# AndrewGYork/rescan_line_sted

Hardware: AMD Instinct MI355X
Metric: simulated frames/s (512x512, 20 RL iters) (higher is better)
Workload: dtype f32; 1 GPU; astronaut 128->512x512 (np.kron x4), point-descan STED PSF 107x107 (2.0x operating point), simulate (H + Philox Poisson) + 20 RL iterations per frame; n_psf=1, rl_iters=20, fft=576x576

## Files before the change

include/rlsted.h:

```cpp
#ifndef RLSTED_H
#define RLSTED_H

#include <stddef.h>
#include <stdint.h>

#ifdef __cplusplus
extern "C" {
#endif

#define RL_OK 0
#define RL_ERR_INVALID -1
#define RL_ERR_HIP -2
#define RL_ERR_UNSUPPORTED -3
#define RL_ERR_STATE -4

#define RL_F32 0
#define RL_F64 1

#define RL_RNG_NONE 0
#define RL_RNG_PHILOX 1

typedef struct rl_ctx rl_ctx;
typedef struct rl_deconv rl_deconv;
typedef struct rl_comm rl_comm;
// ... 46 lines not shown
int rl_deconv_get_noiseless(rl_deconv* h, double* out);
int rl_deconv_get_measurement(rl_deconv* h, double* out);
int rl_deconv_get_estimate(rl_deconv* h, double* out);
int rl_deconv_get_normalization(rl_deconv* h, double* out);

int rl_forward(rl_deconv* h, const double* x, double* out);
int rl_adjoint(rl_deconv* h, const double* y, double* out, int normalize);

int rl_deconv_last_ms(const rl_deconv* h, double* iterate_ms, double* simulate_ms);

int rl_deconv_bench_cycles(rl_deconv* h, int k, int reps, int rng_kind, uint64_t seed, double* total_ms);

int rl_deconv_device_ptr(rl_deconv* h, int which, void** ptr, size_t* n_elements, int* dtype);

int rl_deconv_measurement_written(rl_deconv* h);

int rl_deconv_strategy(const rl_deconv* h, int* separable, int* real_psf_spectrum, int* split_column_pass, int* frame_pairs);

int rl_deconv_object_classes(const rl_deconv* h, int* classes, int* shared_slices, int* slices);

int rl_deconv_simulated_images(const rl_deconv* h, int* images);

int rl_deconv_draws_ahead(const rl_deconv* h, int* slices);

int rl_deconv_unresolved(rl_deconv* h, unsigned long long* count, int reset);

int rl_deconv_dims(const rl_deconv* h, int* batch, int* n_psf, int* ny, int* nx);

typedef struct rl_task {
    const double* object;
    double total_brightness;
    uint64_t seed;
    uint32_t image_id;
} rl_task;
int rl_batch_run(rl_deconv* h, const rl_task* tasks, int n_tasks, int k_iters, int rng_kind, double* estimates_out);

int rl_batch_submit(rl_deconv* h, const rl_task* tasks, int n_tasks, int k_iters, int rng_kind, void* dev_out, int out_dtype);

#define RL_TRACE_FIELDS 6
int rl_batch_submit_checkpoints(rl_deconv* h, const rl_task* tasks, int n_tasks, const int* k_list, int n_k, int rng_kind,
                                void* const* dev_out, int out_dtype, double* const* trace_dev);

int rl_device_alloc(rl_ctx* ctx, size_t bytes, void** dev_out);
int rl_device_free(rl_ctx* ctx, void* dev);
int rl_device_download(rl_ctx* ctx, const void* dev, int dtype, size_t n_elements, double* host_out);
int rl_device_upload(rl_ctx* ctx, void* dev, int dtype, size_t n_elements, const double* host);
// ... 132 lines not shown
```

rescan_line_sted_amd/_lib.py:

```python
import ctypes
import os

import numpy as np

_HERE = os.path.dirname(os.path.abspath(__file__))
LIB_PATH = os.environ.get('RLSTED_LIB') or os.path.join(_HERE, '_lib', 'librlsted.so')
DEFAULT_DEVICE = int(os.environ.get('RLSTED_DEVICE', '0'))

RL_F32, RL_F64 = 0, 1
RNG_NONE, RNG_PHILOX = 0, 1
DTYPES = {'f32': RL_F32, 'float32': RL_F32, 'f64': RL_F64, 'float64': RL_F64}
RL_ACCEL_NONE, RL_ACCEL_BIGGS_ANDREWS = 0, 1
ACCELERATIONS = {None: RL_ACCEL_NONE, 'none': RL_ACCEL_NONE, 'biggs-andrews': RL_ACCEL_BIGGS_ANDREWS}
RL_STOP_DISCREPANCY, RL_STOP_RELATIVE = 1, 2
STOP_RULES = {'discrepancy': RL_STOP_DISCREPANCY, 'relative': RL_STOP_RELATIVE}


def accel_mode(acceleration):
    try:
        return ACCELERATIONS[acceleration]
    except (KeyError, TypeError):
        raise ValueError("acceleration must be None or 'biggs-andrews'; got %r" % (acceleration,)) from None


# ... 33 lines not shown
    'rl_deconv_get_alpha': (_i, [_vp, _dp]),
    'rl_deconv_set_tv': (_i, [_vp, _c.c_double, _c.c_double]),
    'rl_deconv_get_tv': (_i, [_vp, _dp, _dp]),
    'rl_deconv_divergence': (_i, [_vp, _dp]),
    'rl_deconv_iterate_until': (_i, [_vp, _i, _i, _i, _c.c_double, _c.POINTER(_i), _dp, _c.POINTER(_i)]),
    'rl_deconv_get_object': (_i, [_vp, _dp]),
    'rl_deconv_get_noiseless': (_i, [_vp, _dp]),
    'rl_deconv_get_measurement': (_i, [_vp, _dp]),
    'rl_deconv_get_estimate': (_i, [_vp, _dp]),
    'rl_deconv_get_normalization': (_i, [_vp, _dp]),
    'rl_forward': (_i, [_vp, _dp, _dp]),
    'rl_adjoint': (_i, [_vp, _dp, _dp, _i]),
    'rl_deconv_last_ms': (_i, [_vp, _dp, _dp]),
    'rl_deconv_bench_cycles': (_i, [_vp, _i, _i, _i, _c.c_uint64, _dp]),
    'rl_deconv_time_kernels': (_i, [_vp, _i, _dp]),
    'rl_deconv_time_cycle': (_i, [_vp, _i, _i, _c.c_uint64, _dp, _dp, _dp]),
    'rl_deconv_device_ptr': (_i, [_vp, _i, _c.POINTER(_vp), _c.POINTER(_c.c_size_t), _c.POINTER(_i)]),
    'rl_host_alloc': (_i, [_c.c_size_t, _c.POINTER(_vp)]),
    'rl_host_free': (_i, [_vp]),
    'rl_deconv_strategy': (_i, [_vp, _c.POINTER(_i), _c.POINTER(_i), _c.POINTER(_i), _c.POINTER(_i)]),
    'rl_deconv_object_classes': (_i, [_vp, _c.POINTER(_i), _c.POINTER(_i), _c.POINTER(_i)]),
    'rl_deconv_simulated_images': (_i, [_vp, _c.POINTER(_i)]),
    'rl_deconv_draws_ahead': (_i, [_vp, _c.POINTER(_i)]),
    'rl_deconv_unresolved': (_i, [_vp, _c.POINTER(_c.c_uint64), _i]),
    'rl_deconv_dims': (_i, [_vp, _c.POINTER(_i), _c.POINTER(_i), _c.POINTER(_i), _c.POINTER(_i)]),
    'rl_batch_run': (_i, [_vp, _vp, _i, _i, _i, _dp]),
    'rl_batch_submit': (_i, [_vp, _vp, _i, _i, _i, _vp, _i]),
    'rl_batch_submit_checkpoints': (_i, [_vp, _vp, _i, _c.POINTER(_i), _i, _i, _c.POINTER(_vp), _i, _c.POINTER(_vp)]),
    'rl_device_alloc': (_i, [_vp, _c.c_size_t, _c.POINTER(_vp)]),
    'rl_device_free': (_i, [_vp, _vp]),
    'rl_device_download': (_i, [_vp, _vp, _i, _c.c_size_t, _dp]),
    'rl_device_upload': (_i, [_vp, _vp, _i, _c.c_size_t, _dp]),
    'rl_comm_gather_device': (_i, [_vp, _vp, _c.POINTER(_c.c_size_t), _i, _i, _vp]),
    'rl_comm_bcast_host': (_i, [_vp, _dp, _c.c_size_t, _i]),
    'rl_comm_unique_id': (_i, [_vp]),
    'rl_comm_create': (_i, [_vp, _i, _i, _vp, _c.POINTER(_vp)]),
    'rl_comm_destroy': (_i, [_vp]),
    'rl_comm_info': (_i, [_vp, _c.POINTER(_i), _c.POINTER(_i)]),
    'rl_comm_barrier': (_i, [_vp]),
    'rl_comm_allreduce_max': (_i, [_vp, _dp]),
    'rl_gather': (_i, [_vp, _vp, _i, _i, _c.POINTER(_i), _dp]),
    'rl_gather_device': (_i, [_vp, _vp, _i, _i, _c.POINTER(_i), _c.POINTER(_vp), _c.POINTER(_c.c_size_t), _c.POINTER(_i)]),
    'rl_comm_gather_host': (_i, [_vp, _dp, _c.POINTER(_c.c_size_t), _i, _dp]),
    'rl_rotate_image': (_i, [_vp, _dp, _dp, _i, _i, _c.c_double, _i]),
    'rl_fig3_scan': (_i, [_vp, _vp, _dp, _dp, _c.POINTER(_i), _i, _c.POINTER(_i), _i, _dp, _dp, _dp, _dp]),
    'rl_gauss_fit': (_i, [_dp, _i, _dp, _c.POINTER(_i)]),
# ... 162 lines not shown
        return {'ly': ly.value, 'lx': lx.value, 'pitch': pitch.value, 'device_bytes': nbytes.value}

    def strategy(self):
        a, b, c, d = _i(), _i(), _i(), _i()
        check(lib.rl_deconv_strategy(self.handle, ctypes.byref(a), ctypes.byref(b), ctypes.byref(c), ctypes.byref(d)))
        return {'separable': a.value == 1, 'direct_stencil': a.value == 2, 'real_psf_spectrum': bool(b.value),
                'split_column_pass': bool(c.value), 'frame_pairs': bool(d.value)}

    def object_classes(self):
        a, b, c = _i(), _i(), _i()
        check(lib.rl_deconv_object_classes(self.handle, ctypes.byref(a), ctypes.byref(b), ctypes.byref(c)))
        return {'classes': a.value, 'shared_slices': b.value, 'slices': c.value}

    def simulated_images(self):
        a = _i()
        check(lib.rl_deconv_simulated_images(self.handle, ctypes.byref(a)))
        return a.value

    def draws_ahead(self):
        a = _i()
        check(lib.rl_deconv_draws_ahead(self.handle, ctypes.byref(a)))
        return a.value

    def set_object(self, obj, total_brightness=None):
        obj = as_f64(obj).reshape(self.B, self.ny, self.nx)
        tb = None
        if total_brightness is not None:
            tb = as_f64(np.broadcast_to(np.asarray(total_brightness, dtype=np.float64), (self.B,)))
        check(lib.rl_deconv_set_object(self.handle, ptr(obj), ptr(tb) if tb is not None else None))

    def simulate(self, seed=0, rng=RNG_PHILOX):
        check(lib.rl_deconv_simulate(self.handle, rng, _c.c_uint64(seed)))

    def unresolved(self, reset=False):
        n = _c.c_uint64(0)
        check(lib.rl_deconv_unresolved(self.handle, _c.byref(n), 1 if reset else 0))
        return int(n.value)

    def set_measurement(self, noisy):
        noisy = as_f64(noisy).reshape(self.B, self.V, self.ny, self.nx)
        check(lib.rl_deconv_set_measurement(self.handle, ptr(noisy)))

    def measurement_written(self):
        check(lib.rl_deconv_measurement_written(self.handle))

    def iterate(self, k=1):
# ... 175 lines not shown
```

rescan_line_sted_amd/csrc/aux_kernels.hip:

```cpp
#include <hip/hip_runtime.h>
#include <type_traits>
#include "aux_kernels.hpp"
#include "philox_poisson.hpp"

namespace rl {

template <typename T>
__global__ void k_fill(T* p, size_t n, T value) {
    for (size_t i = (size_t)blockIdx.x * blockDim.x + threadIdx.x; i < n; i += (size_t)gridDim.x * blockDim.x) p[i] = value;
}

__global__ void k_psf_dft_rows(const double* __restrict__ psf, const double2* __restrict__ wx, double2* __restrict__ s1,
                               int py, int px, int lx, int kx) {
    const int k = blockIdx.x * blockDim.x + threadIdx.x;
    const int a = blockIdx.y, v = blockIdx.z;
    if (k >= kx) return;
    const int cx = (px - 1) / 2;
    const double* row = psf + ((size_t)v * py + a) * px;
    double re = 0.0, im = 0.0;
    for (int b = 0; b < px; ++b) {
        const int off = ((b - cx) % lx + lx) % lx;
        const double2 w = wx[(int)(((long long)k * off) % lx)];
        re += row[b] * w.x;
        im += row[b] * w.y;
    }
    s1[((size_t)v * py + a) * kx + k] = make_double2(re, im);
// ... 2 lines not shown
template <typename T>
__global__ void k_psf_dft_cols(const double2* __restrict__ s1, const double2* __restrict__ wy, cx<T>* __restrict__ out,
                               int py, int ly, int kx, int pitch, double scale, int transposed) {
    const int k = blockIdx.x * blockDim.x + threadIdx.x;
    const int ky = blockIdx.y, v = blockIdx.z;
    if (k >= pitch) return;
    const int cy = (py - 1) / 2;
    double re = 0.0, im = 0.0;
    if (k < kx) {
        for (int a = 0; a < py; ++a) {
            const int off = ((a - cy) % ly + ly) % ly;
            const double2 w = wy[(int)(((long long)ky * off) % ly)];
            const double2 s = s1[((size_t)v * py + a) * kx + k];
            re += s.x * w.x - s.y * w.y;
            im += s.x * w.y + s.y * w.x;
        }
    }
    if (transposed) {
        if (k < kx) out[((size_t)v * kx + k) * ly + ky] = mk<T>((T)(re * scale), (T)(im * scale));
    } else {
        out[((size_t)v * ly + ky) * pitch + k] = mk<T>((T)(re * scale), (T)(im * scale));
    }
}

struct PoissonKeys {
    unsigned long long seed0;
    unsigned image0, V;
    const unsigned long long* frame_seeds;
    const unsigned* frame_ids;
    const unsigned* rate_frame;
    __device__ __forceinline__ unsigned long long seed(unsigned img) const { return frame_seeds ? frame_seeds[img / V] : seed0; }
    __device__ __forceinline__ unsigned image(unsigned img) const {
        return frame_seeds ? frame_ids[img / V] * V + img % V : image0 + img;
    }
    template <typename T>
    __device__ __forceinline__ T rate(const T* __restrict__ noiseless, unsigned i, unsigned n_pix) const {
        if (!rate_frame) return noiseless[i];
        const unsigned img = i / n_pix, pix = i - img * n_pix;
        return noiseless[((size_t)rate_frame[img / V] * V + img % V) * n_pix + pix];
    }
    template <typename T>
    __device__ __forceinline__ const T* image_rates(const T* __restrict__ noiseless, unsigned img, unsigned n_pix) const {
        return noiseless + (rate_frame ? (size_t)rate_frame[img / V] * V + img % V : (size_t)img) * n_pix;
    }
};

constexpr int kPoissonE = 8, kPoissonTile = 256 * kPoissonE;
template <typename T, bool TILE_IMG>
__global__ void __launch_bounds__(256) k_poisson(const T* __restrict__ noiseless, T* __restrict__ noisy, unsigned n_pix, unsigned total,
                                                 PoissonKeys keys, int rng_kind) {
    __shared__ unsigned lst_idx[2][kPoissonTile];
    __shared__ T lst_lam[2][kPoissonTile];
    __shared__ unsigned cnt[2], cnt_small;
    const unsigned tid = threadIdx.x;
    const unsigned n_tiles = (total + (unsigned)kPoissonTile - 1u) / (unsigned)kPoissonTile;
    const unsigned turn = (unsigned)((float)gridDim.x * 0.6180339887f) | 1u;
    for (unsigned first = 0, round = 0; first < n_tiles; first += gridDim.x, ++round) {
        const unsigned tile = first + (blockIdx.x + round * turn) % gridDim.x;
        if (tile >= n_tiles) continue;
        const unsigned tile0 = tile * (unsigned)kPoissonTile;
        if (tid == 0) cnt[0] = cnt_small = 0;
        __syncthreads();
        const unsigned img_t = TILE_IMG ? tile0 / n_pix : 0u;
        const T* __restrict__ rates_t = TILE_IMG ? keys.image_rates(noiseless, img_t, n_pix) : nullptr;
#pragma unroll
        for (int e = 0; e < kPoissonE; ++e) {
            const unsigned i = tile0 + tid + 256u * (unsigned)e;
            if (i < total) {
// ... 35 lines not shown
                double k;
                const bool done = philox_ptrs_attempt((double)lam_t, (unsigned)seed, (unsigned)(seed >> 32), keys.image(img), pix, blk, &k);
                if (done || last) {
                    noisy[i] = (T)((done || k >= 0.0 ? k : 0.0) + 1e-9);
                } else {
                    const unsigned q2 = atomicAdd(&cnt[cur ^ 1], 1u);
                    lst_idx[cur ^ 1][q2] = i;
                    lst_lam[cur ^ 1][q2] = lam_t;
                }
            }
            __syncthreads();
            n = cnt[cur ^ 1];
            cur ^= 1;
        }
        for (unsigned q = tid; q < n_small; q += 256u) {
            const unsigned at = kPoissonTile - 1u - q, i = lst_idx[0][at];
            const unsigned img = TILE_IMG ? img_t : i / n_pix;
            noisy[i] = (T)(philox_poisson((double)lst_lam[0][at], keys.seed(img), keys.image(img), i - img * n_pix) + 1e-9);
        }
        __syncthreads();
    }
}

template <typename T>
__global__ void __launch_bounds__(1024) k_frame_sums(const T* __restrict__ x, size_t n, double* __restrict__ out) {
    __shared__ double part[16];
    const size_t chunks = gridDim.y, len = (n + chunks - 1) / chunks, i0 = blockIdx.y * len, i1 = i0 + len < n ? i0 + len : n;
    const T* f = x + (size_t)blockIdx.x * n;
    double v = 0.0;
    for (size_t i = i0 + threadIdx.x; i < i1; i += blockDim.x) v += (double)f[i];
    for (int off = 32; off > 0; off >>= 1) v += __shfl_down(v, off, 64);
    if ((threadIdx.x & 63) == 0) part[threadIdx.x >> 6] = v;
    __syncthreads();
    if (threadIdx.x < 64) {
        v = threadIdx.x < (blockDim.x >> 6) ? part[threadIdx.x] : 0.0;
        for (int off = 8; off > 0; off >>= 1) v += __shfl_down(v, off, 64);
        if (threadIdx.x == 0) out[(size_t)blockIdx.x * chunks + blockIdx.y] = v;
    }
}
template <typename T>
static void frame_sums(const T* x, size_t n, size_t frames, double* sums, hipStream_t s) {
    if (n >= ((size_t)1 << 20) && frames * kSumChunks <= 8192) {
        double* part = sums + frames;
        k_frame_sums<T><<<dim3((unsigned)frames, kSumChunks), 1024, 0, s>>>(x, n, part);
        k_frame_sums<double><<<dim3((unsigned)frames, 1), 64, 0, s>>>(part, (size_t)kSumChunks, sums);
    } else {
// ... 66 lines not shown
    const unsigned g = blocks_for(n, 256);
    if (dtype == DT_F32) k_split_real<float><<<g, 256, 0, s>>>((const cx<float>*)z, n, (float*)re, stats);
    else k_split_real<double><<<g, 256, 0, s>>>((const cx<double>*)z, n, (double*)re, stats);
    return hipGetLastError();
}

template <typename T>
__global__ void k_box_norm(const double* __restrict__ integ, T* __restrict__ out, int V, int py, int px, int ny, int nx) {
    const int j = blockIdx.x * blockDim.x + threadIdx.x, i = blockIdx.y;
    if (j >= nx) return;
    out[(size_t)i * nx + j] = box_norm_pixel<T>(integ, V, py, px, ny, nx, i, j);
}

hipError_t aux_box_norm(int dtype, const double* integral_dev, void* out, int V, int py, int px, int ny, int nx, hipStream_t s) {
    const dim3 grid((unsigned)((nx + 255) / 256), (unsigned)ny);
    if (dtype == DT_F32) k_box_norm<float><<<grid, 256, 0, s>>>(integral_dev, (float*)out, V, py, px, ny, nx);
    else k_box_norm<double><<<grid, 256, 0, s>>>(integral_dev, (double*)out, V, py, px, ny, nx);
    return hipGetLastError();
}

hipError_t aux_poisson(int dtype, const void* noiseless, void* noisy, unsigned n_pix, unsigned n_img, unsigned image0,
                       unsigned long long seed, int rng_kind, void* list_ws, hipStream_t s,
                       const unsigned long long* frame_seeds, const unsigned* frame_ids, unsigned V, const unsigned* rate_frame,
                       unsigned grid_cap) {
    (void)list_ws;
    const PoissonKeys keys{seed, image0, V ? V : 1u, frame_seeds, frame_ids, rate_frame};
    const size_t total = (size_t)n_pix * n_img;
    if (total >= 0xffffffffull - (size_t)kPoissonTile * kPoissonGrid) return hipErrorInvalidValue;
    if (total == 0) return hipSuccess;
    const size_t tiles = (total + kPoissonTile - 1) / kPoissonTile;
    const size_t cap = grid_cap < 1 ? 1 : grid_cap > kPoissonGrid ? kPoissonGrid : grid_cap;
    const unsigned g = (unsigned)(tiles > cap ? cap : tiles);
    const bool tile_img = n_pix % (unsigned)kPoissonTile == 0;
    auto launch = [&](auto zero, auto in_image) {
        using T = decltype(zero);
        k_poisson<T, decltype(in_image)::value><<<g, 256, 0, s>>>((const T*)noiseless, (T*)noisy, n_pix, (unsigned)total, keys, rng_kind);
    };
    if (dtype == DT_F32) tile_img ? launch(0.0f, std::true_type{}) : launch(0.0f, std::false_type{});
    else tile_img ? launch(0.0, std::true_type{}) : launch(0.0, std::false_type{});
    return hipGetLastError();
}

hipError_t aux_scale_convert(int dtype, const double* src, void* dst, size_t n, size_t frames, const double* target,
                             double* sums, hipStream_t s, bool want_sums) {
    if (target || want_sums) frame_sums<double>(src, n, frames, sums, s);
    const unsigned g = blocks_for(n * frames, 256);
    if (dtype == DT_F32) k_scale_convert<float><<<g, 256, 0, s>>>(src, (float*)dst, n, frames, target, sums);
    else k_scale_convert<double><<<g, 256, 0, s>>>(src, (double*)dst, n, frames, target, sums);
    return hipGetLastError();
}

template <typename T>
__global__ void k_any_negative(const T* __restrict__ x, size_t n, int* __restrict__ flag) {
    bool neg = false;
    for (size_t i = (size_t)blockIdx.x * blockDim.x + threadIdx.x; i < n; i += (size_t)gridDim.x * blockDim.x) neg = neg || x[i] < (T)0;
// ... 81 lines not shown
```

rescan_line_sted_amd/csrc/aux_kernels.hpp:

```cpp
#pragma once
#include "fft_core.hpp"

#include <cstddef>

#if defined(__HIPCC__) || defined(__HIP_PLATFORM_AMD__)
#include <hip/hip_runtime.h>
#include "kernel_table.hpp"
#endif

namespace rl {

template <typename T>
RL_HD T box_norm_pixel(const double* __restrict__ integ, int V, int py, int px, int ny, int nx, int i, int j) {
    const int cy = (py - 1) / 2, cx = (px - 1) / 2;
    const int a0 = i + cy - ny + 1 > 0 ? i + cy - ny + 1 : 0, a1 = (i + cy < py - 1 ? i + cy : py - 1) + 1;
    const int b0 = j + cx - nx + 1 > 0 ? j + cx - nx + 1 : 0, b1 = (j + cx < px - 1 ? j + cx : px - 1) + 1;
    double acc = 0.0;
    if (a1 > a0 && b1 > b0) {
        for (int v = 0; v < V; ++v) {
            const double* I = integ + (size_t)v * (py + 1) * (px + 1);
            const double s = (I[(size_t)a1 * (px + 1) + b1] - I[(size_t)a0 * (px + 1) + b1]) - (I[(size_t)a1 * (px + 1) + b0] - I[(size_t)a0 * (px + 1) + b0]);
            acc += s > 0.0 ? s : 0.0;
        }
    }
    return (T)acc;
}

#if defined(__HIPCC__) || defined(__HIP_PLATFORM_AMD__)
hipError_t aux_fill(int dtype, void* p, size_t n, double value, hipStream_t s);
hipError_t aux_psf_spectrum(int dtype, const double* psf_dev, const void* wx_dev, const void* wy_dev, void* s1_dev,
                            void* out, int n_psf, int py, int px, int ly, int lx, int kx, int pitch, int transposed,
                            hipStream_t s);
size_t aux_poisson_workspace_bytes(size_t total_pixels);
constexpr unsigned kPoissonGrid = 4096;
hipError_t aux_poisson(int dtype, const void* noiseless, void* noisy, unsigned n_pix, unsigned n_img, unsigned image0,
                       unsigned long long seed, int rng_kind, void* list_ws, hipStream_t s,
                       const unsigned long long* frame_seeds = nullptr, const unsigned* frame_ids = nullptr, unsigned V = 1,
                       const unsigned* rate_frame = nullptr, unsigned grid_cap = kPoissonGrid);
constexpr size_t kSumChunks = 64;
inline size_t aux_sums_elems(size_t frames) { return frames * (1 + kSumChunks); }
hipError_t aux_scale_convert(int dtype, const double* src, void* dst, size_t n, size_t frames, const double* target,
                             double* sums, hipStream_t s, bool want_sums = false);
hipError_t aux_any_negative(int dtype, const void* src, size_t n, int* flag, hipStream_t s);
hipError_t aux_image_sums(int dtype, const void* src, size_t n, size_t frames, double* sums, hipStream_t s);
hipError_t aux_scale_convert_indexed(int dtype, const double* src, const unsigned* idx, size_t n_unique, void* dst, size_t n, size_t frames,
                                     const double* target, double* sums, hipStream_t s);
hipError_t aux_to_f64(int dtype, const void* src, double* dst, size_t total, hipStream_t s);
hipError_t aux_cast(int dtype_src, const void* src, int dtype_dst, void* dst, size_t total, hipStream_t s);
hipError_t aux_gather_images(int dtype, const void* src, void* dst, const unsigned* list, size_t n, size_t images, unsigned V, hipStream_t s);
hipError_t aux_split_real(int dtype, const void* z, size_t n, void* re, double* stats, hipStream_t s);
hipError_t aux_box_norm(int dtype, const double* integral_dev, void* out, int V, int py, int px, int ny, int nx, hipStream_t s);
#endif
}
```

rescan_line_sted_amd/csrc/philox_poisson.hpp:

```cpp
#pragma once
#include <stdint.h>
#include "fft_core.hpp"

#if defined(__clang__)
#define RL_FP_STRICT _Pragma("clang fp contract(off)")
#else
#define RL_FP_STRICT
#endif

namespace rl {

struct Philox4 {
    uint32_t x[4];
};

RL_HD Philox4 philox4x32_10(uint32_t c0, uint32_t c1, uint32_t c2, uint32_t c3, uint32_t k0, uint32_t k1) {
    const uint32_t M0 = 0xD2511F53u, M1 = 0xCD9E8D57u, W0 = 0x9E3779B9u, W1 = 0xBB67AE85u;
#pragma unroll
    for (int r = 0; r < 10; ++r) {
        const uint64_t p0 = (uint64_t)M0 * c0, p1 = (uint64_t)M1 * c2;
        const uint32_t hi0 = (uint32_t)(p0 >> 32), lo0 = (uint32_t)p0;
        const uint32_t hi1 = (uint32_t)(p1 >> 32), lo1 = (uint32_t)p1;
        c0 = hi1 ^ c1 ^ k0;
        c1 = lo1;
// ... 65 lines not shown
    p = p * r + 1.0;
    p = p * r + 1.0;
    DblBits b;
    b.u = (uint64_t)(1023 + (int)n) << 52;
    return p * b.d;
}

RL_HD double det_logfact(double k) {
    RL_FP_STRICT
    if (k < 20.5) {
        double f = 1.0;
        for (int i = 2; i <= (int)k; ++i) f = f * (double)i;
        return det_log(f);
    }
    const double x = k + 1.0;
    const double xi = 1.0 / x, x2 = xi * xi;
    double c = -1.0 / 1680.0;
    c = c * x2 + 1.0 / 1260.0;
    c = c * x2 - 1.0 / 360.0;
    c = c * x2 + 1.0 / 12.0;
    return ((x - 0.5) * det_log(x) - x) + 0.9189385332046727 + c * xi;
}

RL_HD bool philox_poisson_fast(double lam, uint64_t seed, uint32_t image, uint32_t pixel, double* out) {
    RL_FP_STRICT
    if (!(lam > 0.0)) {
        *out = 0.0;
        return true;
    }
    if (lam < 10.0) return false;
    const uint32_t k0 = (uint32_t)seed, k1 = (uint32_t)(seed >> 32);
    const double slam = __builtin_sqrt(lam);
    const double b = 0.931 + 2.53 * slam;
    const double a = -0.059 + 0.02483 * b;
    const double vr = 0.9277 - 3.6224 / (b - 2.0);
    const Philox4 o = philox4x32_10(pixel, image, 0u, 0x504F4953u, k0, k1);
    const double U = u53(o.x[0], o.x[1]) - 0.5;
    const double V = u53(o.x[2], o.x[3]);
    const double us = 0.5 - (U < 0.0 ? -U : U);
    const double k = __builtin_floor((2.0 * a / us + b) * U + lam + 0.43);
    *out = k;
    return us >= 0.07 && V <= vr;
}

RL_HD bool philox_ptrs_attempt(double lam, uint32_t k0, uint32_t k1, uint32_t image, uint32_t pixel, uint32_t blk, double* kout) {
    RL_FP_STRICT
    const double slam = __builtin_sqrt(lam);
    const double b = 0.931 + 2.53 * slam;
    const double a = -0.059 + 0.02483 * b;
    const double vr = 0.9277 - 3.6224 / (b - 2.0);
    const Philox4 o = philox4x32_10(pixel, image, blk, 0x504F4953u, k0, k1);
    const double U = u53(o.x[0], o.x[1]) - 0.5;
    const double V = u53(o.x[2], o.x[3]);
    const double us = 0.5 - (U < 0.0 ? -U : U);
    const double k = __builtin_floor((2.0 * a / us + b) * U + lam + 0.43);
    *kout = k;
    if (us >= 0.07 && V <= vr) return true;
    if (k < 0.0 || (us < 0.013 && V > us)) return false;
    if (!(V > 0.0)) return true;
    const double invalpha = 1.1239 + 1.1328 / (b - 3.4);
    const double loglam = det_log(lam);
    const double lhs = (det_log(V) + det_log(invalpha)) - det_log(a / (us * us) + b);
    const double rhs = (k * loglam - lam) - det_logfact(k);
    return lhs <= rhs;
}

constexpr uint32_t kPoissonMaxBlocks = 64;

RL_HD double philox_poisson(double lam, uint64_t seed, uint32_t image, uint32_t pixel) {
    RL_FP_STRICT
    const uint32_t k0 = (uint32_t)seed, k1 = (uint32_t)(seed >> 32);
    if (!(lam > 0.0)) return 0.0;
    if (lam < 10.0) {
        const double enlam = det_exp(-lam);
        double X = 0.0, prod = 1.0;
        for (uint32_t blk = 0; blk < kPoissonMaxBlocks; ++blk) {
            const Philox4 o = philox4x32_10(pixel, image, blk, 0x504F4953u, k0, k1);
            prod = prod * u53(o.x[0], o.x[1]);
            if (!(prod > enlam)) return X;
            X = X + 1.0;
            prod = prod * u53(o.x[2], o.x[3]);
            if (!(prod > enlam)) return X;
            X = X + 1.0;
        }
        return X;
    }
    double k = 0.0;
// ... 7 lines not shown
```

rescan_line_sted_amd/csrc/rlsted.cpp:

```cpp
#include "../../include/rlsted.h"

#include <hip/hip_runtime.h>

#include <cmath>
#include <cstdio>
#include <cstdlib>
#include <algorithm>
#include <cstring>
#include <map>
#include <string>
#include <vector>

#include "accel_kernels.hpp"
#include "aux_kernels.hpp"
#include "checkpoint_kernels.hpp"
#include "conv_kernels.hpp"
#include "cycle_schedule.hpp"
#include "kernel_table.hpp"
#include "object_classes.hpp"
#include "ctx.hpp"
#include "sep_kernels.hpp"
#include "sep_taps.hpp"
#include "stop_kernels.hpp"
#include "tv_kernels.hpp"
// ... 23 lines not shown

const KernelTable* table_for(int L) {
    switch (L) {
        case 64: return table_64();
        case 192: return table_192();
        case 256: return table_256();
        case 576: return table_576();
        case 1152: return table_1152();
        case 2304: return table_2304();
        case 4608: return table_4608();
    }
    return nullptr;
}
const int kLengths[] = {64, 192, 256, 576, 1152, 2304, 4608};

size_t esize(int dtype) { return dtype == RL_F32 ? 4 : 8; }

struct PlanOptions {
    bool chunk_mb_set = false;
    double chunk_mb = 0;
    int lanes = 2;
    bool draw_ahead = false;
    int draw_grid = 128;
    bool inplace = true;
    int col_order = 4;
    bool pair = false;
    double pair_max_ratio = 4.0;
    bool sub_one = false;
    int fuse_views = -1;
    bool col_split = true;
    bool real_psf = true;
    bool ones_shortcut = true;
    bool share_objects = true;
    int sep = 1;
    int sep_one = 1;
    int direct = 1;
    bool q_exp_est_set = false, q_exp_ratio_set = false;
    int q_exp_est = 14, q_exp_ratio = 14;
};

PlanOptions plan_options(int dtype, int n_psf) {
    PlanOptions o;
    auto flag = [](const char* name, bool unset) {
        const char* s = getenv(name);
        return s ? atoi(s) != 0 : unset;
    };
    auto number = [](const char* name, int unset, bool* set = nullptr) {
        const char* s = getenv(name);
        if (set) *set = s != nullptr;
        return s ? atoi(s) : unset;
    };
    if (const char* s = getenv("RLSTED_CHUNK_MB")) {
        o.chunk_mb_set = true;
        o.chunk_mb = atof(s);
    }
    o.lanes = std::min(std::max(number("RLSTED_LANES", o.lanes), 1), kMaxLanes);
    o.draw_ahead = flag("RLSTED_DRAW_AHEAD", o.draw_ahead);
    o.draw_grid = std::min(std::max(number("RLSTED_DRAW_GRID", o.draw_grid), 1), (int)kPoissonGrid);
    o.inplace = flag("RLSTED_INPLACE", o.inplace);
    o.col_order = std::max(number("RLSTED_COL_ORDER", o.col_order), 1);
    o.pair = flag("RLSTED_PAIR", dtype == RL_F32 && n_psf == 1);
    if (const char* s = getenv("RLSTED_PAIR_MAX_RATIO")) o.pair_max_ratio = atof(s);
    o.sub_one = flag("RLSTED_SUB_ONE", dtype == RL_F32 && RL_SPEC_QUANT == 0);
    if (const char* s = getenv("RLSTED_FUSE_VIEWS")) o.fuse_views = atoi(s) != 0 ? 1 : 0;
    o.col_split = flag("RLSTED_COL_SPLIT", o.col_split);
    o.real_psf = flag("RLSTED_REAL_PSF", o.real_psf);
    o.ones_shortcut = flag("RLSTED_ONES_SHORTCUT", o.ones_shortcut);
    o.share_objects = flag("RLSTED_SHARE_OBJECTS", o.share_objects);
    o.sep = number("RLSTED_SEP", o.sep);
    o.sep_one = number("RLSTED_SEP_ONE", o.sep_one);
    o.direct = number("RLSTED_DIRECT", o.direct);
    o.q_exp_est = number("RLSTED_Q_EXP_EST", o.q_exp_est, &o.q_exp_est_set);
    o.q_exp_ratio = number("RLSTED_Q_EXP_RATIO", o.q_exp_ratio, &o.q_exp_ratio_set);
    return o;
}

struct TempBuffers {
    std::vector<void*> bufs;
    int get(void** p, size_t bytes) {
        HIP_TRY(hipMalloc(p, bytes));
        bufs.push_back(*p);
// ... 665 lines not shown
    }
    int forward_slice(int f0, int nf) { return forward_frames(f0, nf, off(obj, (size_t)f0 * n_img()), off(noiseless, (size_t)f0 * V * n_img())); }
    int forward_frames(int f0, int nf, const void* x, void* out) {
        if (sep) return sep_forward(x, out, off(sep_tmp(), (size_t)f0 * V * n_img()), nf);
        void* sb = off(spec_b, (size_t)f0 * V * n_spec() * 2);
        void* sa = !pair ? off(spec_a, (size_t)f0 * n_spec() * 2) : sb;
        return forward_pass(x, out, nf, sa, sb, col_split() ? parked(f0) : nullptr);
    }
    std::vector<int> obj_class;
    int n_classes = 0;
    std::vector<SliceShare> share_slices;
    int share_cf = 0;
    std::vector<uint32_t> share_reps, share_rate;
    struct ShareLists { const unsigned *rep_frames, *rate_of; };
    ShareLists share_lists{nullptr, nullptr};
    unsigned* share_dev = nullptr;
    void *obj_c = nullptr, *noiseless_c = nullptr;
    void *cls_spec_a = nullptr, *cls_spec_b = nullptr, *cls_spec_x = nullptr;
    size_t share_cap = 0;
    int share_classes = 0;
    int last_sim_images = 0;
    bool noiseless_sparse = false;
    int last_shared_slices = 0, last_slices = 0;
    int last_draws_ahead = 0;
    bool share_possible() const { return opt.share_objects && !sep && (int)obj_class.size() == B && n_classes < B; }
    size_t layout_share(int cf) {
        share_cf = 0;
        noiseless_sparse = false;
        share_classes = 0;
        share_layout(obj_class, cf, share_slices, share_reps, share_rate);
        return (size_t)class_layout(obj_class, cf, share_slices, share_reps, share_rate);
    }
    int build_share(int cf, const ShareLists* staged) { return place_share(cf, layout_share(cf), staged); }
    int place_share(int cf, size_t total, const ShareLists* staged) {
        if (total > share_cap) {
            HIP_TRY(hipDeviceSynchronize());
            share_cap = 0;
            RL_TRY(release(&obj_c));
            RL_TRY(release(&noiseless_c));
            RL_TRY(release(&cls_spec_a));
            RL_TRY(release(&cls_spec_b));
            RL_TRY(release(&cls_spec_x));
            const size_t cap = (total + 7) / 8 * 8, sp = n_spec() * 2 * esize(dtype);
            RL_TRY(alloc(&obj_c, cap * n_img() * esize(dtype), SLACK));
            RL_TRY(alloc(&noiseless_c, cap * V * n_img() * esize(dtype), SLACK));
            if (!pair_layout) RL_TRY(alloc(&cls_spec_a, cap * sp, SLACK));
// ... 76 lines not shown
        return RL_OK;
    }
    struct Run { int k; bool restart; const Draw* draw; const Checkpoints* cp; int cf; };
    hipStream_t stream_of(int s) const { return s == kCtxStream ? ctx->stream : lane[s].stream; }
    hipEvent_t event_of(const StreamOp& op) const {
        const Lane& l = lane[op.lane];
        switch (op.event) {
            case EventKind::FORK: return fork;
            case EventKind::RATES_READY: return rates_ready;
            case EventKind::DONE: return l.done;
            case EventKind::DRAWN: return l.drawn;
            case EventKind::BEGUN: return l.begun;
            case EventKind::DRAWN_AHEAD: return l.drawn_ahead;
            case EventKind::NONE: break;
        }
        return nullptr;
    }
    int draw_slice(const Draw& d, int sl, int f0, int nf, bool shared, bool ahead) {
        void* ws = ahead ? nullptr : (char*)slice_ws + (size_t)sl * slice_ws_stride;
        TimedScope t(this, TK_POISSON, false);
        const hipError_t e = aux_poisson(dtype, shared ? noiseless_c : off(noiseless, (size_t)f0 * V * n_img()), off(meas, (size_t)f0 * V * n_img()),
                                         (unsigned)n_img(), (unsigned)(nf * V), (unsigned)(f0 * V), d.seed, d.rng_kind, ws, cur(),
                                         d.key_seeds ? d.key_seeds + f0 : nullptr, d.key_ids ? d.key_ids + f0 : nullptr, (unsigned)V,
                                         shared ? share_lists.rate_of + f0 : nullptr, ahead ? (unsigned)opt.draw_grid : (unsigned)kPoissonGrid);
        return e == hipSuccess ? RL_OK : fail(RL_ERR_HIP, std::string("Poisson kernels: ") + hipGetErrorString(e));
    }
    int loop_slice(const Run& r, int f0, int nf) {
        const int k = r.k;
        const bool restart = r.restart;
        const bool shortcut = restart && opt.ones_shortcut && spec_ones && k > 0 && !sep;
        const bool ones_first = shortcut && !accel && !tv_on();
        if (restart && !ones_first) RL_TRY(start_estimate_chunk(f0, nf, !shortcut));
        const bool drop = pair && k >= 4;
        int cp_next = 0;
        for (int i = 0; i < k; ++i) {
            if (accel) RL_TRY(accel_step(f0, nf, acc_steps + i, shortcut && i == 0, restart && i == 0));
            else if (tv_on()) RL_TRY(tv_iterate({f0, nf, shortcut && i == 0, restart && i == 0,  pair}, i > 0 || tv_sum_valid, true));
            else RL_TRY(iterate_chunk({f0, nf, shortcut && i == 0, restart && i == 0, drop && i == k - 1, ones_first && i == 0}));
            if (r.cp && cp_next < r.cp->n_k && r.cp->k_list[cp_next] == i + 1) RL_TRY(take_checkpoint(*r.cp, cp_next++, f0, nf));
        }
        return RL_OK;
    }
    int enqueue(const StreamOp& op, const Run& r) {
        const int f0 = op.slice * r.cf, nf = f0 + r.cf <= B ? r.cf : B - f0;
        active = stream_of(op.stream);
        switch (op.op) {
            case OpKind::WAIT: HIP_TRY(hipStreamWaitEvent(active, event_of(op), 0)); return RL_OK;
// ... 21 lines not shown
        in.share_classes = share_classes;
        in.share_slices = share_slices.data();
        in.draw_ahead = opt.draw_ahead;
        in.cycle_follows = cycle_follows;
        in.before = cycle_state;
        cycle_schedule(in, schedule);
        if (schedule.forks) RL_TRY(ensure_lanes());
        if (draw) {
            const size_t stride = (aux_poisson_workspace_bytes((size_t)cf * V * n_img()) + 255) / 256 * 256;
            if (slice_ws_bytes < stride * schedule.slices) {
                HIP_TRY(hipDeviceSynchronize());
                slice_ws_bytes = 0;
                RL_TRY(release(&slice_ws));
                RL_TRY(alloc(&slice_ws, stride * schedule.slices));
                slice_ws_bytes = stride * schedule.slices;
            }
            slice_ws_stride = stride;
        }
        struct ActiveGuard {
            hipStream_t& a;
            ~ActiveGuard() { a = nullptr; }
        } active_guard{active};
        const Run run{k, restart, draw, cp, cf};
        int rc = RL_OK;
        for (const StreamOp& op : schedule.ops) {
            if (rc != RL_OK && !op.join) continue;
            const int r = enqueue(op, run);
            if (rc == RL_OK) rc = r;
        }
        active = nullptr;
        if (rc != RL_OK) {
            const std::string keep = rl::last_error();
            if (!schedule.joins) (void)join_lanes();
            cycle_state = CycleState{};
            rl::last_error() = keep;
            return rc;
        }
        cycle_state = schedule.after;
        if (draw) {
            last_draws_ahead = schedule.draws_ahead;
            noiseless_sparse = schedule.shared_slices > 0;
            last_shared_slices = schedule.shared_slices;
            last_slices = schedule.slices;
            last_sim_images = schedule.sim_images;
        }
        if (restart) {
            est_ready = true;
            spec_valid = true;
            iterations = 0;
        }
        if (pair && k >= 4) spec_valid = false;
        if (accel) {
            spec_valid = false;
            acc_steps += k;
        }
        if (tv_on()) spec_valid = false;
        if (k > 0 || restart) tv_sum_valid = tv_on() && !accel && k > 0;
        iterations += k;
        return RL_OK;
    }
};

namespace rl {
// ... 602 lines not shown
}


int rl_deconv_strategy(const rl_deconv* h, int* separable, int* real_psf_spectrum, int* split_column_pass, int* frame_pairs) {
    if (!h) return fail(RL_ERR_INVALID, "handle is NULL");
    if (frame_pairs) *frame_pairs = h->pair ? 1 : 0;
    if (separable) *separable = h->sep ? (h->sep_direct ? 2 : 1) : 0;
    if (real_psf_spectrum) *real_psf_spectrum = h->psf_hat_re ? 1 : 0;
    if (split_column_pass) *split_column_pass = !h->sep && !h->pair && h->col_split() ? 1 : 0;
    return RL_OK;
}

int rl_deconv_object_classes(const rl_deconv* h, int* classes, int* shared_slices, int* slices) {
    if (!h) return fail(RL_ERR_INVALID, "handle is NULL");
    if (classes) *classes = (int)h->obj_class.size() == h->B ? h->n_classes : 0;
    if (shared_slices) *shared_slices = h->last_shared_slices;
    if (slices) *slices = h->last_slices;
    return RL_OK;
}

int rl_deconv_draws_ahead(const rl_deconv* h, int* slices) {
    if (!h || !slices) return fail(RL_ERR_INVALID, "NULL argument");
    *slices = h->last_draws_ahead;
    return RL_OK;
}

int rl_deconv_simulated_images(const rl_deconv* h, int* images) {
    if (!h || !images) return fail(RL_ERR_INVALID, "NULL argument");
    *images = h->last_sim_images;
    return RL_OK;
}

int rl_deconv_unresolved(rl_deconv* h, unsigned long long* count, int reset) {
    if (!h || !count) return fail(RL_ERR_INVALID, "NULL argument");
    HIP_TRY(hipSetDevice(h->ctx->device));
    HIP_TRY(hipMemcpyAsync(count, h->unresolved, sizeof(unsigned long long), hipMemcpyDeviceToHost, h->ctx->stream));
    if (reset) HIP_TRY(hipMemsetAsync(h->unresolved, 0, sizeof(unsigned long long), h->ctx->stream));
    HIP_TRY(hipStreamSynchronize(h->ctx->stream));
    return RL_OK;
}

int rl_deconv_dims(const rl_deconv* h, int* batch, int* n_psf, int* ny, int* nx) {
    if (!h) return fail(RL_ERR_INVALID, "handle is NULL");
    if (batch) *batch = h->B;
    if (n_psf) *n_psf = h->V;
    if (ny) *ny = h->ny;
// ... 325 lines not shown
```

Measured before the change: 21910 frames/s.

## Add grouped Poisson draw kernel sharing rate setup across frames of one object class

Adds a Poisson sampling kernel for shared-object batches. It processes groups of frames that share a noiseless rate image, computes the PTRS per-pixel constants once into LDS, and compacts rejected draws into LDS work lists that are retried in rounds. It is enabled by default only when rate_frame sharing and Philox are active. The goal is to cut repeated rate reads, repeated transcendental setup and divergent rejection loops, at the cost of heavy LDS use, many workgroup barriers and reduced occupancy.

```diff
diff --git a/include/rlsted.h b/include/rlsted.h
--- a/include/rlsted.h
+++ b/include/rlsted.h
@@ -92,6 +92,8 @@
 int rl_deconv_simulated_images(const rl_deconv* h, int* images);
 
 int rl_deconv_draws_ahead(const rl_deconv* h, int* slices);
+
+int rl_deconv_grouped_draws(const rl_deconv* h, int* slices);
 
 int rl_deconv_unresolved(rl_deconv* h, unsigned long long* count, int reset);
 
diff --git a/rescan_line_sted_amd/_lib.py b/rescan_line_sted_amd/_lib.py
--- a/rescan_line_sted_amd/_lib.py
+++ b/rescan_line_sted_amd/_lib.py
@@ -79,6 +79,7 @@
     'rl_deconv_object_classes': (_i, [_vp, _c.POINTER(_i), _c.POINTER(_i), _c.POINTER(_i)]),
     'rl_deconv_simulated_images': (_i, [_vp, _c.POINTER(_i)]),
     'rl_deconv_draws_ahead': (_i, [_vp, _c.POINTER(_i)]),
+    'rl_deconv_grouped_draws': (_i, [_vp, _c.POINTER(_i)]),
     'rl_deconv_unresolved': (_i, [_vp, _c.POINTER(_c.c_uint64), _i]),
     'rl_deconv_dims': (_i, [_vp, _c.POINTER(_i), _c.POINTER(_i), _c.POINTER(_i), _c.POINTER(_i)]),
     'rl_batch_run': (_i, [_vp, _vp, _i, _i, _i, _dp]),
@@ -287,6 +288,11 @@
         check(lib.rl_deconv_draws_ahead(self.handle, ctypes.byref(a)))
         return a.value
 
+    def grouped_draws(self):
+        a = _i()
+        check(lib.rl_deconv_grouped_draws(self.handle, ctypes.byref(a)))
+        return a.value
+
     def set_object(self, obj, total_brightness=None):
         obj = as_f64(obj).reshape(self.B, self.ny, self.nx)
         tb = None
diff --git a/rescan_line_sted_amd/csrc/aux_kernels.hip b/rescan_line_sted_amd/csrc/aux_kernels.hip
--- a/rescan_line_sted_amd/csrc/aux_kernels.hip
+++ b/rescan_line_sted_amd/csrc/aux_kernels.hip
@@ -1,7 +1,9 @@
 #include <hip/hip_runtime.h>
 #include <type_traits>
 #include "aux_kernels.hpp"
+#include "dev_sync.hpp"
 #include "philox_poisson.hpp"
+#include "poisson_kernels.hpp"
 
 namespace rl {
 
@@ -50,28 +52,6 @@
         out[((size_t)v * ly + ky) * pitch + k] = mk<T>((T)(re * scale), (T)(im * scale));
     }
 }
-
-struct PoissonKeys {
-    unsigned long long seed0;
-    unsigned image0, V;
-    const unsigned long long* frame_seeds;
-    const unsigned* frame_ids;
-    const unsigned* rate_frame;
-    __device__ __forceinline__ unsigned long long seed(unsigned img) const { return frame_seeds ? frame_seeds[img / V] : seed0; }
-    __device__ __forceinline__ unsigned image(unsigned img) const {
-        return frame_seeds ? frame_ids[img / V] * V + img % V : image0 + img;
-    }
-    template <typename T>
-    __device__ __forceinline__ T rate(const T* __restrict__ noiseless, unsigned i, unsigned n_pix) const {
-        if (!rate_frame) return noiseless[i];
-        const unsigned img = i / n_pix, pix = i - img * n_pix;
-        return noiseless[((size_t)rate_frame[img / V] * V + img % V) * n_pix + pix];
-    }
-    template <typename T>
-    __device__ __forceinline__ const T* image_rates(const T* __restrict__ noiseless, unsigned img, unsigned n_pix) const {
-        return noiseless + (rate_frame ? (size_t)rate_frame[img / V] * V + img % V : (size_t)img) * n_pix;
-    }
-};
 
 constexpr int kPoissonE = 8, kPoissonTile = 256 * kPoissonE;
 template <typename T, bool TILE_IMG>
@@ -153,6 +133,15 @@
     }
 }
 
+struct PoissonSync : DevSync {
+    __device__ __forceinline__ unsigned lds_add(unsigned* p, unsigned v) const { return atomicAdd(p, v); }
+};
+template <typename T>
+__global__ void __launch_bounds__(kPoissonGroupPix) __attribute__((amdgpu_waves_per_eu(5))) k_poisson_groups(PoissonGroupParams<T> p) {
+    __shared__ __attribute__((aligned(8))) unsigned char lds[kPoissonGroupLds];
+    poisson_groups_body<T>(p, threadIdx.x, blockIdx.x, gridDim.x, lds, PoissonSync{});
+}
+
 template <typename T>
 __global__ void __launch_bounds__(1024) k_frame_sums(const T* __restrict__ x, size_t n, double* __restrict__ out) {
     __shared__ double part[16];
@@ -265,7 +254,7 @@
 hipError_t aux_poisson(int dtype, const void* noiseless, void* noisy, unsigned n_pix, unsigned n_img, unsigned image0,
                        unsigned long long seed, int rng_kind, void* list_ws, hipStream_t s,
                        const unsigned long long* frame_seeds, const unsigned* frame_ids, unsigned V, const unsigned* rate_frame,
-                       unsigned grid_cap) {
+                       unsigned grid_cap, bool groups) {
     (void)list_ws;
     const PoissonKeys keys{seed, image0, V ? V : 1u, frame_seeds, frame_ids, rate_frame};
     const size_t total = (size_t)n_pix * n_img;
@@ -274,6 +263,13 @@
     const size_t tiles = (total + kPoissonTile - 1) / kPoissonTile;
     const size_t cap = grid_cap < 1 ? 1 : grid_cap > kPoissonGrid ? kPoissonGrid : grid_cap;
     const unsigned g = (unsigned)(tiles > cap ? cap : tiles);
+    if (aux_poisson_groups(groups, rng_kind, rate_frame != nullptr)) {
+        const unsigned items = poisson_group_items(n_pix, n_img / keys.V, keys.V);
+        const unsigned gg = (unsigned)(items > cap ? cap : items);
+        if (dtype == DT_F32) k_poisson_groups<float><<<gg, kPoissonGroupPix, 0, s>>>(PoissonGroupParams<float>{(const float*)noiseless, (float*)noisy, n_pix, n_img / keys.V, keys});
+        else k_poisson_groups<double><<<gg, kPoissonGroupPix, 0, s>>>(PoissonGroupParams<double>{(const double*)noiseless, (double*)noisy, n_pix, n_img / keys.V, keys});
+        return hipGetLastError();
+    }
     const bool tile_img = n_pix % (unsigned)kPoissonTile == 0;
     auto launch = [&](auto zero, auto in_image) {
         using T = decltype(zero);
diff --git a/rescan_line_sted_amd/csrc/aux_kernels.hpp b/rescan_line_sted_amd/csrc/aux_kernels.hpp
--- a/rescan_line_sted_amd/csrc/aux_kernels.hpp
+++ b/rescan_line_sted_amd/csrc/aux_kernels.hpp
@@ -33,10 +33,11 @@
                             hipStream_t s);
 size_t aux_poisson_workspace_bytes(size_t total_pixels);
 constexpr unsigned kPoissonGrid = 4096;
+inline bool aux_poisson_groups(bool groups, int rng_kind, bool rate_frame) { return groups && rate_frame && rng_kind == 1; }
 hipError_t aux_poisson(int dtype, const void* noiseless, void* noisy, unsigned n_pix, unsigned n_img, unsigned image0,
                        unsigned long long seed, int rng_kind, void* list_ws, hipStream_t s,
                        const unsigned long long* frame_seeds = nullptr, const unsigned* frame_ids = nullptr, unsigned V = 1,
-                       const unsigned* rate_frame = nullptr, unsigned grid_cap = kPoissonGrid);
+                       const unsigned* rate_frame = nullptr, unsigned grid_cap = kPoissonGrid, bool groups = true);
 constexpr size_t kSumChunks = 64;
 inline size_t aux_sums_elems(size_t frames) { return frames * (1 + kSumChunks); }
 hipError_t aux_scale_convert(int dtype, const double* src, void* dst, size_t n, size_t frames, const double* target,
diff --git a/rescan_line_sted_amd/csrc/philox_poisson.hpp b/rescan_line_sted_amd/csrc/philox_poisson.hpp
--- a/rescan_line_sted_amd/csrc/philox_poisson.hpp
+++ b/rescan_line_sted_amd/csrc/philox_poisson.hpp
@@ -111,6 +111,61 @@
     return ((x - 0.5) * det_log(x) - x) + 0.9189385332046727 + c * xi;
 }
 
+struct PtrsRate {
+    double lam, b, a, vr;
+};
+RL_HD PtrsRate ptrs_rate(double lam) {
+    RL_FP_STRICT
+    PtrsRate r;
+    const double slam = __builtin_sqrt(lam);
+    r.lam = lam;
+    r.b = 0.931 + 2.53 * slam;
+    r.a = -0.059 + 0.02483 * r.b;
+    r.vr = 0.9277 - 3.6224 / (r.b - 2.0);
+    return r;
+}
+struct PtrsSlow {
+    double loglam, log_invalpha;
+};
+RL_HD PtrsSlow ptrs_slow(const PtrsRate& r) {
+    RL_FP_STRICT
+    PtrsSlow s;
+    const double invalpha = 1.1239 + 1.1328 / (r.b - 3.4);
+    s.loglam = det_log(r.lam);
+    s.log_invalpha = det_log(invalpha);
+    return s;
+}
+struct PtrsCandidate {
+    double U, V, us, k;
+};
+RL_HD Philox4 ptrs_block(uint32_t k0, uint32_t k1, uint32_t image, uint32_t pixel, uint32_t blk) {
+    return philox4x32_10(pixel, image, blk, 0x504F4953u, k0, k1);
+}
+RL_HD PtrsCandidate ptrs_candidate(const PtrsRate& r, const Philox4& o) {
+    RL_FP_STRICT
+    PtrsCandidate c;
+    c.U = u53(o.x[0], o.x[1]) - 0.5;
+    c.V = u53(o.x[2], o.x[3]);
+    c.us = 0.5 - (c.U < 0.0 ? -c.U : c.U);
+    c.k = __builtin_floor((2.0 * r.a / c.us + r.b) * c.U + r.lam + 0.43);
+    return c;
+}
+RL_HD bool ptrs_squeeze(const PtrsRate& r, const PtrsCandidate& c) {
+    RL_FP_STRICT
+    return c.us >= 0.07 && c.V <= r.vr;
+}
+template <class Slow>
+RL_HD bool ptrs_accept(const PtrsRate& r, const PtrsCandidate& c, Slow slow) {
+    RL_FP_STRICT
+    if (ptrs_squeeze(r, c)) return true;
+    if (c.k < 0.0 || (c.us < 0.013 && c.V > c.us)) return false;
+    if (!(c.V > 0.0)) return true;
+    const PtrsSlow s = slow();
+    const double lhs = (det_log(c.V) + s.log_invalpha) - det_log(r.a / (c.us * c.us) + r.b);
+    const double rhs = (c.k * s.loglam - r.lam) - det_logfact(c.k);
+    return lhs <= rhs;
+}
+
 RL_HD bool philox_poisson_fast(double lam, uint64_t seed, uint32_t image, uint32_t pixel, double* out) {
     RL_FP_STRICT
     if (!(lam > 0.0)) {
@@ -118,40 +173,18 @@
         return true;
     }
     if (lam < 10.0) return false;
-    const uint32_t k0 = (uint32_t)seed, k1 = (uint32_t)(seed >> 32);
-    const double slam = __builtin_sqrt(lam);
-    const double b = 0.931 + 2.53 * slam;
-    const double a = -0.059 + 0.02483 * b;
-    const double vr = 0.9277 - 3.6224 / (b - 2.0);
-    const Philox4 o = philox4x32_10(pixel, image, 0u, 0x504F4953u, k0, k1);
-    const double U = u53(o.x[0], o.x[1]) - 0.5;
-    const double V = u53(o.x[2], o.x[3]);
-    const double us = 0.5 - (U < 0.0 ? -U : U);
-    const double k = __builtin_floor((2.0 * a / us + b) * U + lam + 0.43);
-    *out = k;
-    return us >= 0.07 && V <= vr;
+    const PtrsRate r = ptrs_rate(lam);
+    const PtrsCandidate c = ptrs_candidate(r, ptrs_block((uint32_t)seed, (uint32_t)(seed >> 32), image, pixel, 0u));
+    *out = c.k;
+    return ptrs_squeeze(r, c);
 }
 
 RL_HD bool philox_ptrs_attempt(double lam, uint32_t k0, uint32_t k1, uint32_t image, uint32_t pixel, uint32_t blk, double* kout) {
     RL_FP_STRICT
-    const double slam = __builtin_sqrt(lam);
-    const double b = 0.931 + 2.53 * slam;
-    const double a = -0.059 + 0.02483 * b;
-    const double vr = 0.9277 - 3.6224 / (b - 2.0);
-    const Philox4 o = philox4x32_10(pixel, image, blk, 0x504F4953u, k0, k1);
-    const double U = u53(o.x[0], o.x[1]) - 0.5;
-    const double V = u53(o.x[2], o.x[3]);
-    const double us = 0.5 - (U < 0.0 ? -U : U);
-    const double k = __builtin_floor((2.0 * a / us + b) * U + lam + 0.43);
-    *kout = k;
-    if (us >= 0.07 && V <= vr) return true;
-    if (k < 0.0 || (us < 0.013 && V > us)) return false;
-    if (!(V > 0.0)) return true;
-    const double invalpha = 1.1239 + 1.1328 / (b - 3.4);
-    const double loglam = det_log(lam);
-    const double lhs = (det_log(V) + det_log(invalpha)) - det_log(a / (us * us) + b);
-    const double rhs = (k * loglam - lam) - det_logfact(k);
-    return lhs <= rhs;
+    const PtrsRate r = ptrs_rate(lam);
+    const PtrsCandidate c = ptrs_candidate(r, ptrs_block(k0, k1, image, pixel, blk));
+    *kout = c.k;
+    return ptrs_accept(r, c, [&r]() { return ptrs_slow(r); });
 }
 
 constexpr uint32_t kPoissonMaxBlocks = 64;
diff --git a/rescan_line_sted_amd/csrc/poisson_kernels.hpp b/rescan_line_sted_amd/csrc/poisson_kernels.hpp
--- /dev/null
+++ b/rescan_line_sted_amd/csrc/poisson_kernels.hpp
@@ -0,0 +1,166 @@
+#pragma once
+#include <stddef.h>
+#include <stdint.h>
+#include "philox_poisson.hpp"
+
+namespace rl {
+
+struct PoissonKeys {
+    unsigned long long seed0;
+    unsigned image0, V;
+    const unsigned long long* frame_seeds;
+    const unsigned* frame_ids;
+    const unsigned* rate_frame;
+    RL_HD unsigned long long frame_seed(unsigned f) const { return frame_seeds ? frame_seeds[f] : seed0; }
+    RL_HD unsigned frame_image(unsigned f, unsigned view) const { return (frame_seeds ? frame_ids[f] * V : image0 + f * V) + view; }
+    RL_HD unsigned long long seed(unsigned img) const { return frame_seeds ? frame_seeds[img / V] : seed0; }
+    RL_HD unsigned image(unsigned img) const { return frame_seeds ? frame_ids[img / V] * V + img % V : image0 + img; }
+    template <typename T>
+    RL_HD T rate(const T* __restrict__ noiseless, unsigned i, unsigned n_pix) const {
+        if (!rate_frame) return noiseless[i];
+        const unsigned img = i / n_pix, pix = i - img * n_pix;
+        return noiseless[((size_t)rate_frame[img / V] * V + img % V) * n_pix + pix];
+    }
+    template <typename T>
+    RL_HD const T* image_rates(const T* __restrict__ noiseless, unsigned img, unsigned n_pix) const {
+        return noiseless + (rate_frame ? (size_t)rate_frame[img / V] * V + img % V : (size_t)img) * n_pix;
+    }
+};
+
+constexpr int kPoissonGroup = 8, kPoissonGroupPix = 256, kPoissonGroupDraws = kPoissonGroup * kPoissonGroupPix;
+constexpr int kPoissonGroupTab = 6;
+constexpr size_t kPoissonGroupLds = 2 * kPoissonGroupDraws * sizeof(unsigned) + kPoissonGroupTab * kPoissonGroupPix * sizeof(double) + (4 + 3 * kPoissonGroup) * sizeof(unsigned) + kPoissonGroupPix;
+
+template <typename T>
+struct PoissonGroupParams {
+    const T* noiseless;
+    T* noisy;
+    unsigned n_pix, frames;
+    PoissonKeys keys;
+};
+RL_HD unsigned poisson_group_items(unsigned n_pix, unsigned frames, unsigned V) {
+    return (frames + kPoissonGroup - 1u) / kPoissonGroup * V * ((n_pix + kPoissonGroupPix - 1u) / kPoissonGroupPix);
+}
+
+template <typename T, class Sync>
+RL_HD void poisson_groups_body(const PoissonGroupParams<T>& p, unsigned tid, unsigned bx, unsigned grid, unsigned char* lds_raw, const Sync& sync) {
+    unsigned* const lst0 = reinterpret_cast<unsigned*>(lds_raw);
+    unsigned* const lst1 = lst0 + kPoissonGroupDraws;
+    double* const tab = reinterpret_cast<double*>(lst1 + kPoissonGroupDraws);
+    unsigned* const cnt = reinterpret_cast<unsigned*>(tab + kPoissonGroupTab * kPoissonGroupPix);
+    unsigned* const key = cnt + 4;
+    unsigned char* const ord = reinterpret_cast<unsigned char*>(key + 3 * kPoissonGroup);
+    const PoissonKeys& keys = p.keys;
+    const unsigned V = keys.V, n_pix = p.n_pix;
+    const bool sorted = p.frames <= (unsigned)kPoissonGroupPix;
+    if (sorted) {
+        if (tid < p.frames) lst0[tid] = keys.rate_frame[tid];
+        sync.wg();
+        if (tid < p.frames) {
+            const unsigned c = lst0[tid];
+            unsigned place = 0;
+            for (unsigned f = 0; f < p.frames; ++f) {
+                const unsigned cf = lst0[f];
+                place += (cf < c || (cf == c && f < tid)) ? 1u : 0u;
+            }
+            ord[place] = (unsigned char)tid;
+        }
+        sync.wg();
+    }
+    auto frame_at = [ord, sorted](unsigned j) { return sorted ? (unsigned)ord[j] : j; };
+    const unsigned tiles = (n_pix + kPoissonGroupPix - 1u) / kPoissonGroupPix;
+    const unsigned n_items = poisson_group_items(n_pix, p.frames, V);
+    const unsigned turn = (unsigned)((float)grid * 0.6180339887f) | 1u;
+    auto table_rate = [tab](unsigned px) {
+        PtrsRate r;
+        r.lam = tab[px];
+        r.b = tab[kPoissonGroupPix + px];
+        r.a = tab[2 * kPoissonGroupPix + px];
+        r.vr = tab[3 * kPoissonGroupPix + px];
+        return r;
+    };
+    for (unsigned first = 0, round = 0; first < n_items; first += grid, ++round) {
+        const unsigned item = first + (bx + round * turn) % grid;
+        if (item >= n_items) continue;
+        const unsigned tile = item % tiles, view = item / tiles % V, g0 = item / (tiles * V) * kPoissonGroup;
+        const unsigned g1 = g0 + kPoissonGroup < p.frames ? g0 + kPoissonGroup : p.frames;
+        const unsigned pix = tile * kPoissonGroupPix + tid;
+        const bool inside = pix < n_pix;
+        if (tid < g1 - g0) {
+            const unsigned long long seed = keys.frame_seed(frame_at(g0 + tid));
+            key[3u * tid] = (unsigned)seed;
+            key[3u * tid + 1u] = (unsigned)(seed >> 32);
+            key[3u * tid + 2u] = keys.frame_image(frame_at(g0 + tid), view);
+        }
+        for (unsigned fa = g0; fa < g1;) {
+            const unsigned cls = keys.rate_frame[frame_at(fa)];
+            unsigned fb = fa + 1;
+            while (fb < g1 && keys.rate_frame[frame_at(fb)] == cls) ++fb;
+            if (tid == 0) cnt[0] = cnt[2] = 0;
+            sync.wg();
+            if (inside) {
+                const T lam_t = p.noiseless[((size_t)cls * V + view) * n_pix + pix];
+                const double lam = (double)lam_t;
+                tab[tid] = lam;
+                if (!(lam > 0.0)) {
+                    for (unsigned f = fa; f < fb; ++f) p.noisy[((size_t)frame_at(f) * V + view) * n_pix + pix] = (T)(0.0 + 1e-9);
+                } else if (lam < 10.0) {
+                    for (unsigned f = fa; f < fb; ++f) lst0[kPoissonGroupDraws - 1u - sync.lds_add(&cnt[2], 1u)] = (f - g0) << 8 | tid;
+                } else {
+                    const PtrsRate r = ptrs_rate(lam);
+                    const PtrsSlow sl = ptrs_slow(r);
+                    tab[kPoissonGroupPix + tid] = r.b;
+                    tab[2 * kPoissonGroupPix + tid] = r.a;
+                    tab[3 * kPoissonGroupPix + tid] = r.vr;
+                    tab[4 * kPoissonGroupPix + tid] = sl.loglam;
+                    tab[5 * kPoissonGroupPix + tid] = sl.log_invalpha;
+                    for (unsigned f = fa; f < fb; ++f) {
+                        const unsigned* const kf = key + 3u * (f - g0);
+                        const PtrsCandidate c = ptrs_candidate(r, ptrs_block(kf[0], kf[1], kf[2], pix, 0u));
+                        if (ptrs_squeeze(r, c)) p.noisy[((size_t)frame_at(f) * V + view) * n_pix + pix] = (T)(c.k + 1e-9);
+                        else lst0[sync.lds_add(&cnt[0], 1u)] = (f - g0) << 8 | tid;
+                    }
+                }
+            }
+            sync.wg();
+            unsigned n = cnt[0];
+            const unsigned n_small = cnt[2];
+            unsigned *cur = lst0, *nxt = lst1;
+            unsigned ci = 0;
+            for (unsigned blk = 0; n > 0; ++blk) {
+                if (tid == 0) cnt[ci ^ 1u] = 0;
+                sync.wg();
+                const bool last = blk + 1 == kPoissonMaxBlocks;
+                for (unsigned q = tid; q < n; q += (unsigned)kPoissonGroupPix) {
+                    const unsigned e = cur[q], px = e & 255u, f = frame_at(g0 + (e >> 8));
+                    const unsigned* const kf = key + 3u * (e >> 8);
+                    const PtrsRate r = table_rate(px);
+                    const PtrsCandidate c = ptrs_candidate(r, ptrs_block(kf[0], kf[1], kf[2], tile * kPoissonGroupPix + px, blk));
+                    const bool done = ptrs_accept(r, c, [tab, px]() {
+                        PtrsSlow s;
+                        s.loglam = tab[4 * kPoissonGroupPix + px];
+                        s.log_invalpha = tab[5 * kPoissonGroupPix + px];
+                        return s;
+                    });
+                    if (done || last) p.noisy[((size_t)f * V + view) * n_pix + tile * kPoissonGroupPix + px] = (T)((done || c.k >= 0.0 ? c.k : 0.0) + 1e-9);
+                    else nxt[sync.lds_add(&cnt[ci ^ 1u], 1u)] = e;
+                }
+                sync.wg();
+                n = cnt[ci ^ 1u];
+                ci ^= 1u;
+                unsigned* const t = cur;
+                cur = nxt;
+                nxt = t;
+            }
+            for (unsigned q = tid; q < n_small; q += (unsigned)kPoissonGroupPix) {
+                const unsigned e = lst0[kPoissonGroupDraws - 1u - q], px = e & 255u, f = frame_at(g0 + (e >> 8));
+                p.noisy[((size_t)f * V + view) * n_pix + tile * kPoissonGroupPix + px] =
+                    (T)(philox_poisson(tab[px], (unsigned long long)key[3u * (e >> 8) + 1u] << 32 | key[3u * (e >> 8)], key[3u * (e >> 8) + 2u], tile * kPoissonGroupPix + px) + 1e-9);
+            }
+            sync.wg();
+            fa = fb;
+        }
+    }
+}
+
+}
diff --git a/rescan_line_sted_amd/csrc/rlsted.cpp b/rescan_line_sted_amd/csrc/rlsted.cpp
--- a/rescan_line_sted_amd/csrc/rlsted.cpp
+++ b/rescan_line_sted_amd/csrc/rlsted.cpp
@@ -69,6 +69,7 @@
     int lanes = 2;
     bool draw_ahead = false;
     int draw_grid = 128;
+    bool poisson_groups = true;
     bool inplace = true;
     int col_order = 4;
     bool pair = false;
@@ -104,6 +105,7 @@
     o.lanes = std::min(std::max(number("RLSTED_LANES", o.lanes), 1), kMaxLanes);
     o.draw_ahead = flag("RLSTED_DRAW_AHEAD", o.draw_ahead);
     o.draw_grid = std::min(std::max(number("RLSTED_DRAW_GRID", o.draw_grid), 1), (int)kPoissonGrid);
+    o.poisson_groups = flag("RLSTED_POISSON_GROUPS", o.poisson_groups);
     o.inplace = flag("RLSTED_INPLACE", o.inplace);
     o.col_order = std::max(number("RLSTED_COL_ORDER", o.col_order), 1);
     o.pair = flag("RLSTED_PAIR", dtype == RL_F32 && n_psf == 1);
@@ -815,6 +817,7 @@
     int last_sim_images = 0;
     bool noiseless_sparse = false;
     int last_shared_slices = 0, last_slices = 0;
+    int grouped_draws = 0, last_grouped_draws = 0;
     int last_draws_ahead = 0;
     bool share_possible() const { return opt.share_objects && !sep && (int)obj_class.size() == B && n_classes < B; }
     size_t layout_share(int cf) {
@@ -937,7 +940,9 @@
         const hipError_t e = aux_poisson(dtype, shared ? noiseless_c : off(noiseless, (size_t)f0 * V * n_img()), off(meas, (size_t)f0 * V * n_img()),
                                          (unsigned)n_img(), (unsigned)(nf * V), (unsigned)(f0 * V), d.seed, d.rng_kind, ws, cur(),
                                          d.key_seeds ? d.key_seeds + f0 : nullptr, d.key_ids ? d.key_ids + f0 : nullptr, (unsigned)V,
-                                         shared ? share_lists.rate_of + f0 : nullptr, ahead ? (unsigned)opt.draw_grid : (unsigned)kPoissonGrid);
+                                         shared ? share_lists.rate_of + f0 : nullptr, ahead ? (unsigned)opt.draw_grid : (unsigned)kPoissonGrid,
+                                         opt.poisson_groups);
+        if (aux_poisson_groups(opt.poisson_groups, d.rng_kind, shared)) ++grouped_draws;
         return e == hipSuccess ? RL_OK : fail(RL_ERR_HIP, std::string("Poisson kernels: ") + hipGetErrorString(e));
     }
     int loop_slice(const Run& r, int f0, int nf) {
@@ -1005,6 +1010,7 @@
             ~ActiveGuard() { a = nullptr; }
         } active_guard{active};
         const Run run{k, restart, draw, cp, cf};
+        grouped_draws = 0;
         int rc = RL_OK;
         for (const StreamOp& op : schedule.ops) {
             if (rc != RL_OK && !op.join) continue;
@@ -1022,6 +1028,7 @@
         cycle_state = schedule.after;
         if (draw) {
             last_draws_ahead = schedule.draws_ahead;
+            last_grouped_draws = grouped_draws;
             noiseless_sparse = schedule.shared_slices > 0;
             last_shared_slices = schedule.shared_slices;
             last_slices = schedule.slices;
@@ -1670,6 +1677,12 @@
 int rl_deconv_draws_ahead(const rl_deconv* h, int* slices) {
     if (!h || !slices) return fail(RL_ERR_INVALID, "NULL argument");
     *slices = h->last_draws_ahead;
+    return RL_OK;
+}
+
+int rl_deconv_grouped_draws(const rl_deconv* h, int* slices) {
+    if (!h || !slices) return fail(RL_ERR_INVALID, "NULL argument");
+    *slices = h->last_grouped_draws;
     return RL_OK;
 }
 
```

After: 22180 frames/s (median of 6 runs). 1.01x the previous value.
